# janinethoma/soft_contrastive_learning

Hardware: AMD Instinct MI355X
Metric: train-step images/sec (VGG16-NetVLAD soft-MS, 640x480) (higher is better)
Workload: dtype bf16; 1 GPU; configs[1]: wms soft-contrastive train step, VGG16-NetVLAD K=64, 24 images/GPU 640x480, bf16 backbone, float32-accurate NetVLAD + f32 loss; global_batch=24, locations=1200, parallelism=dp1, optimizer=adam

## Files before the change

### soft_contrastive_learning_amd/csrc/conv64.hip

```cpp
#include <mutex>

#include "conv_pack_layout.h"
#include "scl_common.h"

namespace {

constexpr int C64 = 64;
constexpr int TH = 8, TW = 32;
constexpr int WR = TH + 2, WC = TW + 2;
constexpr int SCR_LD = 40;
constexpr int SCR = 32 * SCR_LD;


constexpr bool kWrwBufPath = true;

constexpr int kFwSlab = 2048;
constexpr int kFwMaxSlabs = 2 * kSclMaxConvCus;
constexpr size_t kFwAux = (size_t)kFwMaxSlabs * kFwSlab, kFwAuxLen = 256;
constexpr size_t kFwStamps = kFwAux / 2, kFwCorners = kFwAux / 4 * 3;
constexpr int kFwMaxBatch = 8192;
static_assert((size_t)kSclMaxConvCus * kFwSlab <= kFwStamps, "the fused route's slabs (one per CU) end below the stamps");
static_assert(kFwStamps + (size_t)kSclMaxConvCus * 4 * 12 * 2 <= kFwCorners, "the stamps end below the corner copy");
static_assert(kFwCorners + (size_t)kFwMaxBatch * 4 * 64 / 2 <= kFwAux, "the corner copy ends below the border sums");

template <int CIN, int KOUT, int GEO = 0>
struct ConvCfg {
  static_assert(GEO == 0 || (CIN == 64 && KOUT == 64), "GEO 1 is conv1_2's geometry");
  static constexpr int TH_ = (CIN == 64 && GEO == 0) ? 8 : 4;
  static constexpr int WR_ = TH_ + 2;
  static constexpr int PIX = CIN + 8;
  static constexpr int WIN_ = WR_ * WC * PIX;
  static constexpr int PPP = CIN / 8;
  static constexpr int PIECES_ = WR_ * WC * PPP;
  static constexpr int WAVES = (CIN == 64 && KOUT == 64 && GEO == 0) ? 8 : 4;
  static constexpr int NTHR = 64 * WAVES;
  static constexpr int SPP = PPP + 1;
  static constexpr int CHUNKS = (WR_ * WC * SPP + 63) / 64;
  static constexpr int NI = (CHUNKS + WAVES - 1) / WAVES;
  static constexpr int SPT = CIN / 16;
  static constexpr int KS = 9 * SPT;
  static constexpr int NT = KOUT / 32;
  static constexpr int PARTS = WAVES / NT;
  static constexpr int MT = TH_ / PARTS;
  static constexpr size_t LDS =
      (2 * (size_t)WIN_ + WAVES * (size_t)SCR) * sizeof(unsigned short);
};

template <int CIN, int KOUT>
__global__ __launch_bounds__(256) void conv3x3_pack_kernel(const void* __restrict__ w,
                                                           int64_t sk, int64_t sc, int64_t sh,
                                                           int64_t sw, int flags,
                                                           unsigned short* __restrict__ packed) {
  using Cfg = ConvCfg<CIN, KOUT>;
  const int transposed = flags & 1, wf32 = flags & 2;
  const int idx = blockIdx.x * 256 + threadIdx.x;
  if (idx >= Cfg::NT * Cfg::KS * 512) return;
  const int64_t off = pack_src_offset(pack_reg_coord(idx, CIN), sk, sc, sh, sw, transposed);
  packed[idx] = weight_bf16(w, off, wf32);
}

template <int CIN, int KOUT, int EPI, int PL = 0, int FW = 0, int GEO = 0>
__global__ __launch_bounds__((ConvCfg<CIN, KOUT, GEO>::NTHR), (GEO ? 2 : 1)) void conv3x3_kernel(const unsigned short* __restrict__ x,
                                                         const unsigned short* __restrict__ packed,
                                                         int B, int H, int W,
                                                         unsigned short* __restrict__ out,
                                                         const float* __restrict__ bias, int relu,
                                                         unsigned short* __restrict__ pooled,
                                                         const unsigned short* __restrict__ mask,
                                                         unsigned char* __restrict__ pidx,
                                                         const unsigned char* __restrict__ uidx) {
  using Cfg = ConvCfg<CIN, KOUT, GEO>;
  constexpr int TH_ = Cfg::TH_, PIX = Cfg::PIX, WIN_ = Cfg::WIN_, KS = Cfg::KS, MT = Cfg::MT;
  static_assert(!FW || GEO == 0, "the fused first-layer gradients are written for the 8-row tile");
  extern __shared__ __attribute__((aligned(16))) unsigned short lds[];
  const int lane = threadIdx.x & 63, wid = threadIdx.x >> 6;
  const int r = lane & 31, h = lane >> 5;
  const int nt = wid % Cfg::NT, part = wid / Cfg::NT;
  unsigned short* scr = lds + 2 * WIN_ + wid * SCR;
  static_assert(!FW || (CIN == 64 && KOUT == 64 && EPI == 3 && PL == 1), "FW: conv1_2 backward-data only");
  constexpr int FWPL = 32, FGPL = TH * TW * FWPL, FXW = WR * WC * 4;
  float* dwl = reinterpret_cast<float*>(lds + 2 * WIN_ + Cfg::WAVES * SCR);
  unsigned short* xwl = reinterpret_cast<unsigned short*>(dwl + Cfg::WAVES * 1024);
  unsigned short* imc = lds + 2 * WIN_;
  const unsigned short* fx0 = reinterpret_cast<const unsigned short*>(pooled);
  float* fslabs = reinterpret_cast<float*>(pidx);
  const float bias_r = (EPI == 1 || EPI == 2 || EPI == 4) ? bias[32 * nt + r] : 0.f;
  constexpr bool SWAP = EPI == 0 || EPI == 1 || EPI == 3;
  f32x4 bias_q[4];
#pragma unroll
  for (int j = 0; j < 4; ++j)
    bias_q[j] = (SWAP && EPI == 1) ? *reinterpret_cast<const f32x4*>(bias + 32 * nt + 8 * j + 4 * h)
                                   : f32x4{0.f, 0.f, 0.f, 0.f};

  u32x4 wf[KS];
#pragma unroll
  for (int ks = 0; ks < KS; ++ks)
    wf[ks] = *reinterpret_cast<const u32x4*>(packed + (((int64_t)nt * KS + ks) * 64 + lane) * 8);

  const int tiles_x = (W + TW - 1) / TW, tiles_y = (H + TH_ - 1) / TH_;
  const int per_img = tiles_x * tiles_y;
  const int ntiles = B * per_img;

  const int wid_s = __builtin_amdgcn_readfirstlane(wid);
  int rel[Cfg::NI], roff[Cfg::NI];
#pragma unroll
  for (int i = 0; i < Cfg::NI; ++i) {
    const int slot = 64 * (wid_s + Cfg::WAVES * i) + lane;
    const int pix = slot / Cfg::SPP, piece = slot % Cfg::SPP;
    rel[i] = (piece < Cfg::PPP && pix < Cfg::WR_ * WC) ? ((pix / WC) << 8) | (pix % WC) : -1;
    roff[i] = ((pix / WC) * W + pix % WC) * CIN + 8 * piece;
  }
  const unsigned short* zeros = reinterpret_cast<const unsigned short*>(zero_block);
  auto stage_issue = [&](int tile, int buf) {
    const int b = tile / per_img, t2 = tile % per_img;
    const int y0 = (t2 / tiles_x) * TH_ - 1, x0 = (t2 % tiles_x) * TW - 1;
    const int xo = ((b * H + y0) * W + x0) * CIN;
    const unsigned base = lds_byte_of(lds) + buf * WIN_ * 2;
#pragma unroll
    for (int i = 0; i < Cfg::NI; ++i) {
      const int j = wid_s + Cfg::WAVES * i;
      if (j < Cfg::CHUNKS) {
        const int y = y0 + (rel[i] >> 8), xx = x0 + (rel[i] & 255);
        const bool ok = (unsigned)y < (unsigned)H && (unsigned)xx < (unsigned)W;
        const unsigned short* src = ok ? x + (xo + roff[i]) : zeros;
        if (rel[i] >= 0) glds16(src, base + j * 1024);
      }
    }
  };
  constexpr int PWR = TH_ / 2 + 2, PWC = TW / 2 + 2, PPP = Cfg::PPP;
  constexpr int PNR = PL ? (PWR * PWC * PPP + Cfg::NTHR - 1) / Cfg::NTHR : 1;
  constexpr int PLIVE = CIN == 64 ? 1 : PNR, NB = PNR / PLIVE, SPAN = KS / NB;
  static_assert(!PL || (PNR % PLIVE == 0 && 4 * PLIVE + 2 < SPAN), "un-pooling schedule");
  const int Ho = H >> 1, Wo = W >> 1;
  u32x4 pg[PLIVE];
  uint2 pi[PLIVE];
  const int p_piece = threadIdx.x % PPP;
  auto p_rc = [&](int rd) {
    int tid_ = threadIdx.x;
    if (FW || GEO) asm volatile("" : "+v"(tid_));
    const int pp = (tid_ + Cfg::NTHR * rd) / PPP;
    return pp < PWR * PWC ? ((pp / PWC) << 8) | (pp % PWC) : -1;
  };
  auto pool_issue = [&](int tile, int g) {
    const int b = tile / per_img, t2 = tile % per_img;
    const int py0 = (t2 / tiles_x) * (TH_ / 2) - 1, px0 = (t2 % tiles_x) * (TW / 2) - 1;
#pragma unroll
    for (int i = 0; i < PLIVE; ++i) {
      const int rc = p_rc(g * PLIVE + i);
      const int py = py0 + (rc >> 8), px = px0 + (rc & 255);
      const int off = ((b * Ho + py) * Wo + px) * CIN + 8 * p_piece;
      if (rc >= 0 && (unsigned)py < (unsigned)Ho && (unsigned)px < (unsigned)Wo) {
        pg[i] = *reinterpret_cast<const u32x4*>(x + off);
        pi[i] = *reinterpret_cast<const uint2*>(uidx + off);
      } else {
        pg[i] = u32x4{0u, 0u, 0u, 0u};
        pi[i] = uint2{0u, 0u};
      }
    }
  };
  auto pool_write = [&](int g, int i, int pos, int buf) {
    const int rc = p_rc(g * PLIVE + i);
    const int wy = 2 * (rc >> 8) + (pos >> 1) - 1, wx = 2 * (rc & 255) + (pos & 1) - 1;
    const UnpoolFlags fl = unpool_flags(pi[i].x, pi[i].y);
    const u32x4 o = unpool8(pg[i], fl, pos);
    if (rc >= 0 && (unsigned)wy < (unsigned)Cfg::WR_ && (unsigned)wx < (unsigned)WC)
      *reinterpret_cast<u32x4*>(lds + buf * WIN_ + (wy * WC + wx) * PIX + 8 * p_piece) = o;
  };

  const int dbg = SCL_DIAG_ONLY(relu >> 1);
  relu &= 1;
  const short relu_floor = relu ? (short)0 : (short)-32768;
  if ((dbg & 4) && (threadIdx.x >> 6) >= 4) __builtin_amdgcn_s_setprio(1);
  unsigned short xreg[FW ? 2 : 1];
  auto xwin_load = [&](int tile_) {
    const int b_ = tile_ / per_img, t2_ = tile_ % per_img;
    const int ty_ = (t2_ / tiles_x) * TH_, tx_ = (t2_ % tiles_x) * TW;
    int tid2 = threadIdx.x;
    asm volatile("" : "+v"(tid2));
#pragma unroll
    for (int v = 0; v < 2; ++v) {
      const int idx = v * Cfg::NTHR + tid2;
      const int pix = idx / 3, c = idx - 3 * pix;
      const int y = ty_ - 1 + pix / WC, xx = tx_ - 1 + pix % WC;
      const bool ok = idx < 3 * WR * WC && y >= 0 && y < H && xx >= 0 && xx < W;
      xreg[v] = ok ? fx0[(((int64_t)b_ * H + y) * W + xx) * 3 + c] : (unsigned short)0;
    }
  };
  auto xwin_store = [&](int par) {
    int tid2 = threadIdx.x;
    asm volatile("" : "+v"(tid2));
#pragma unroll
    for (int v = 0; v < 2; ++v) {
      const int idx = v * Cfg::NTHR + tid2;
      const int pix = idx / 3, c = idx - 3 * pix;
      if (idx < 3 * WR * WC) xwl[par * FXW + pix * 4 + c] = xreg[v];
    }
  };
  int tile = blockIdx.x;
  if (FW) {
#pragma unroll
    for (int v = 0; v < 4; ++v)
      *reinterpret_cast<f32x4*>(dwl + wid * 1024 + v * 256 + lane * 4) = f32x4{0.f, 0.f, 0.f, 0.f};
    if (tile < ntiles) {
      xwin_load(tile);
      xwin_store(0);
    }
  }
  int xpar = 0;
  uint64_t fstamp[10];
  int ftile = 0;
#define FW_STAMP(k)                                                                     \
  if (FW && (dbg & 64))                                                                 \
  asm volatile("s_memtime %0\n\ts_waitcnt lgkmcnt(0)" : "=s"(fstamp[k])::"memory")
  if (tile < ntiles) {
    if (PL) {
#pragma unroll
      for (int g = 0; g < NB; ++g) {
        pool_issue(tile, g);
#pragma unroll
        for (int sl = 0; sl < 4 * PLIVE; ++sl) pool_write(g, sl >> 2, sl & 3, 0);
      }
    } else {
      stage_issue(tile, 0);
    }
  }
  asm volatile("s_waitcnt vmcnt(0)" ::: "memory");
  __syncthreads();
  int buf = 0;
  for (; tile < ntiles; tile += gridDim.x) {
    FW_STAMP(0);
    const int next = (dbg & 1) ? ntiles : tile + gridDim.x;
    if (next < ntiles) {
      if (PL) pool_issue(next, 0); else stage_issue(next, buf ^ 1);
    }
    u32x4 mk[EPI == 3 ? MT : 1][2];
    if (EPI == 3) {
      const int b_ = tile / per_img, t2_ = tile % per_img;
      const int my0 = (t2_ / tiles_x) * TH_ + MT * part, mx = (t2_ % tiles_x) * TW + (lane >> 1);
#pragma unroll
      for (int mt = 0; mt < MT; ++mt) {
        const bool in_ = my0 + mt < H && mx < W;
        const int64_t mo = (((int64_t)b_ * H + my0 + mt) * W + mx) * KOUT + 32 * nt + 8 * (lane & 1);
        mk[mt][0] = in_ ? *reinterpret_cast<const u32x4*>(mask + mo) : u32x4{0u, 0u, 0u, 0u};
        mk[mt][1] = in_ ? *reinterpret_cast<const u32x4*>(mask + mo + 16) : u32x4{0u, 0u, 0u, 0u};
      }
    }

    const unsigned short* wb = lds + buf * WIN_ + ((MT * part) * WC + r) * PIX + 8 * h;
    f32x16 acc[MT];
#pragma unroll
    for (int mt = 0; mt < MT; ++mt) acc[mt] = zero16();
    constexpr int WRW = MT + 2, NST = Cfg::SPT * WRW * 3, RING = 4, AHEAD = 3;
    auto frag_at = [&](int st) {
      const int c = st / (WRW * 3), wr = (st / 3) % WRW, kw = st % 3;
      return *reinterpret_cast<const u32x4*>(wb + (wr * WC + kw) * PIX + 16 * c);
    };
    u32x4 af[RING];
#pragma unroll
    for (int st = 0; st < AHEAD; ++st) af[st] = frag_at(st);
#pragma unroll
    for (int st = 0; st < NST; ++st) {
      if (st + AHEAD < NST) af[(st + AHEAD) % RING] = frag_at(st + AHEAD);
      __builtin_amdgcn_sched_barrier(0);
      const int c = st / (WRW * 3), wr = (st / 3) % WRW, kw = st % 3;
#pragma unroll
      for (int mt = 0; mt < MT; ++mt) {
        const int kh = wr - mt;
        if (kh >= 0 && kh < 3)
          acc[mt] = SWAP ? mfma32b(wf[(3 * kh + kw) * Cfg::SPT + c], af[st % RING], acc[mt])
                         : mfma32b(af[st % RING], wf[(3 * kh + kw) * Cfg::SPT + c], acc[mt]);
      }
      const int ks = st * KS / NST;
      if (PL && (st == 0 || ks != (st - 1) * KS / NST)) {
        constexpr int W0 = SPAN - 4 * PLIVE - 2;
        const int g = ks / SPAN, kk = ks % SPAN;
        if (kk >= W0 && kk < W0 + 4 * PLIVE) pool_write(g, (kk - W0) >> 2, (kk - W0) & 3, buf ^ 1);
        if (kk == SPAN - 1 && g + 1 < NB && next < ntiles) pool_issue(next, g + 1);
      }
    }

    FW_STAMP(1);
    asm volatile("s_waitcnt vmcnt(0)" ::: "memory");
    FW_STAMP(2);
    if (FW) {
      __syncthreads();
      FW_STAMP(3);
      if (next < ntiles) xwin_load(next);
    }

    const int b = tile / per_img, t2 = tile % per_img;
    const int oy0 = (t2 / tiles_x) * TH_ + MT * part, ox0 = (t2 % tiles_x) * TW;
#pragma unroll
    for (int mt = 0; mt < (EPI == 4 ? 0 : MT); ++mt) {
      const int px = lane >> 1, hf = lane & 1;
      const int oy = oy0 + mt, ox = ox0 + px;
      const bool inside = oy < H && ox < W;
      const int64_t o_off = (((int64_t)b * H + oy) * W + ox) * KOUT + 32 * nt + 8 * hf;
      const u32x4 y0v = mk[EPI == 3 ? mt : 0][0], y1v = mk[EPI == 3 ? mt : 0][1];
      if (SWAP) {
#pragma unroll
        for (int j = 0; j < 4; ++j) {
          f32x4 v = {acc[mt][4 * j], acc[mt][4 * j + 1], acc[mt][4 * j + 2], acc[mt][4 * j + 3]};
          if (EPI == 1) v += bias_q[j];
          unsigned p0 = pack2_bf16(v[0], v[1]), p1 = pack2_bf16(v[2], v[3]);
          if (EPI == 1) {
            p0 = max2_i16(p0, relu_floor);
            p1 = max2_i16(p1, relu_floor);
          }
          *reinterpret_cast<uint2*>(scr + r * SCR_LD + 8 * j + 4 * h) = make_uint2(p0, p1);
        }
      } else {
#pragma unroll
        for (int q = 0; q < 16; ++q) scr[acc_row(q, h) * SCR_LD + r] = f32_to_bf16(acc[mt][q]);
      }
      __builtin_amdgcn_wave_barrier();
      u32x4 v0 = *reinterpret_cast<const u32x4*>(scr + px * SCR_LD + 8 * hf);
      u32x4 v1 = *reinterpret_cast<const u32x4*>(scr + px * SCR_LD + 8 * hf + 16);
      __builtin_amdgcn_wave_barrier();
      if (EPI == 3) {
        v0 = relu_mask(v0, y0v);
        v1 = relu_mask(v1, y1v);
      }
      if (FW && (dbg & 32)) {
      } else if (FW) {
        unsigned short* gzp = lds + buf * WIN_ + nt * FGPL + ((MT * part + mt) * TW + px) * FWPL + 8 * hf;
        *reinterpret_cast<u32x4*>(gzp) = v0;
        *reinterpret_cast<u32x4*>(gzp + 16) = v1;
        const bool cy0 = oy == 0, cy1 = oy == H - 1, cx0 = ox == 0, cx1 = ox == W - 1;
        if ((cy0 || cy1) && (cx0 || cx1)) {
          unsigned short* cp = reinterpret_cast<unsigned short*>(fslabs + kFwCorners) +
                               ((int64_t)b * 4 + (cy1 ? 2 : 0) + (cx1 ? 1 : 0)) * C64 + 32 * nt + 8 * hf;
          *reinterpret_cast<u32x4*>(cp) = v0;
          *reinterpret_cast<u32x4*>(cp + 16) = v1;
        }
      } else if (inside && !(dbg & 2)) {
        *reinterpret_cast<u32x4*>(out + o_off) = v0;
        *reinterpret_cast<u32x4*>(out + o_off + 16) = v1;
      }
    }
    if (FW) {
      FW_STAMP(4);
      __syncthreads();
      FW_STAMP(5);
      int tid2 = threadIdx.x;
      asm volatile("" : "+v"(tid2));
      const unsigned short* xw = xwl + xpar * FXW;
      const int ty_ = oy0 - MT * part, tx_ = ox0;
#pragma unroll
      for (int v = 0; v < ((dbg & 8) ? 0 : 2); ++v) {
        const int u = v * Cfg::NTHR + tid2;
        const int hh = u & 1, n = (u >> 1) & 31, s_ = u >> 6;
        const int row = s_ >> 1, col0 = 16 * (s_ & 1) + 8 * hh;
        const int nc = n < 27 ? n : 26, tap = nc / 3, c = nc - 3 * tap;
        const unsigned short* wp = xw + ((row + tap / 3) * WC + col0 + tap % 3) * 4 + c;
        unsigned e[8];
#pragma unroll
        for (int j = 0; j < 8; ++j) e[j] = wp[4 * j];
        if (n >= 27) {
          const int y = ty_ + row, xb = tx_ + col0;
          const bool rowflag = n == 27 || (n == 28 && y == 0) || (n == 29 && y == H - 1);
          const int colx = n == 30 ? 0 : (n == 31 ? W - 1 : -1);
#pragma unroll
          for (int j = 0; j < 8; ++j) e[j] = (rowflag || xb + j == colx) ? 0x3f80u : 0u;
        }
        *reinterpret_cast<u32x4*>(imc + (s_ * 32 + n) * 16 + 8 * hh) =
            u32x4{e[0] | (e[1] << 16), e[2] | (e[3] << 16), e[4] | (e[5] << 16), e[6] | (e[7] << 16)};
      }
      FW_STAMP(6);
      __syncthreads();
      FW_STAMP(7);
      int lane2 = lane, wid2 = wid;
      asm volatile("" : "+v"(lane2), "+v"(wid2));
      const int mt_ = wid2 & 1, pq = wid2 >> 1;
      const int r2 = lane2 & 31, h2 = lane2 >> 5;
      const int q4 = (lane2 >> 2) & 3, p4 = lane2 & 3, gq = lane2 >> 4;
      const unsigned short* ga = lds + buf * WIN_ + mt_ * FGPL + (8 * (gq >> 1) + q4) * FWPL +
                                 16 * (gq & 1) + 4 * p4;
      f32x16 dacc;
#pragma unroll
      for (int v = 0; v < 4; ++v) {
        const f32x4 t = *reinterpret_cast<const f32x4*>(dwl + wid2 * 1024 + v * 256 + lane2 * 4);
#pragma unroll
        for (int j = 0; j < 4; ++j) dacc[4 * v + j] = t[j];
      }
#pragma unroll
      for (int u = 0; u < ((dbg & 16) ? 0 : 4); ++u) {
        const int s_ = 4 * pq + u;
        const u32x4 a = tr_pair(ga + s_ * 16 * FWPL, 4 * FWPL);
        const u32x4 bfr = *reinterpret_cast<const u32x4*>(imc + (s_ * 32 + r2) * 16 + 8 * h2);
        dacc = mfma32b(a, bfr, dacc);
      }
#pragma unroll
      for (int v = 0; v < 4; ++v)
        *reinterpret_cast<f32x4*>(dwl + wid2 * 1024 + v * 256 + lane2 * 4) =
            f32x4{dacc[4 * v], dacc[4 * v + 1], dacc[4 * v + 2], dacc[4 * v + 3]};
      if (next < ntiles) xwin_store(xpar ^ 1);
      xpar ^= 1;
      FW_STAMP(8);
    }
    if (EPI == 2 || EPI == 4) {
      const int PH2 = H / 2, PW2 = W / 2;
      unsigned char* scr8 = reinterpret_cast<unsigned char*>(scr + 16 * SCR_LD);
#pragma unroll
      for (int mp = 0; mp < MT / 2; ++mp) {
#pragma unroll
        for (int q = 0; q < 16; q += 2) {
          const float m0 = fmaxf(acc[2 * mp][q], acc[2 * mp][q + 1]);
          const float m1 = fmaxf(acc[2 * mp + 1][q], acc[2 * mp + 1][q + 1]);
          const float m = fmaxf(m0, m1);
          scr[(acc_row(q, h) >> 1) * SCR_LD + r] = f32_to_bf16(fmaxf(m + bias_r, 0.f));
          if (EPI == 4) {
            const int k = acc[2 * mp][q] == m ? 0 : acc[2 * mp][q + 1] == m ? 1
                          : acc[2 * mp + 1][q] == m ? 2 : 3;
            scr8[(acc_row(q, h) >> 1) * 32 + r] = (unsigned char)k;
          }
        }
        __builtin_amdgcn_wave_barrier();
        const int px = lane >> 2, qu = lane & 3;
        const u32x4 v = *reinterpret_cast<const u32x4*>(scr + px * SCR_LD + 8 * qu);
        uint2 kv = uint2{0u, 0u};
        if (EPI == 4) kv = *reinterpret_cast<const uint2*>(scr8 + px * 32 + 8 * qu);
        __builtin_amdgcn_wave_barrier();
        const int py = (oy0 >> 1) + mp, pxg = (ox0 >> 1) + px;
        if (py < PH2 && pxg < PW2) {
          const int64_t po = (((int64_t)b * PH2 + py) * PW2 + pxg) * KOUT + 32 * nt + 8 * qu;
          *reinterpret_cast<u32x4*>(pooled + po) = v;
          if (EPI == 4) *reinterpret_cast<uint2*>(pidx + po) = kv;
        }
      }
    }

    __syncthreads();
    if (FW && (dbg & 64)) {
      FW_STAMP(9);
      if ((int)threadIdx.x == 64 * (dbg >> 7) && ftile >= 2 && ftile < 6) {
        uint64_t* o = reinterpret_cast<uint64_t*>(fslabs + kFwStamps) +
                      ((int64_t)blockIdx.x * 4 + (ftile - 2)) * 12;
#pragma unroll
        for (int k = 0; k < 10; ++k) o[k] = fstamp[k];
      }
      ++ftile;
    }
    buf ^= 1;
  }
#undef FW_STAMP
  if (FW) {
    __syncthreads();
    float* red = reinterpret_cast<float*>(lds);
    const int mt_ = wid & 1, pq = wid >> 1;
#pragma unroll
    for (int v = 0; v < 4; ++v) {
      const f32x4 t = *reinterpret_cast<const f32x4*>(dwl + wid * 1024 + v * 256 + lane * 4);
#pragma unroll
      for (int j = 0; j < 4; ++j) red[(pq * 64 + 32 * mt_ + acc_row(4 * v + j, h)) * 32 + r] = t[j];
    }
    __syncthreads();
    for (int e = threadIdx.x; e < kFwSlab; e += Cfg::NTHR)
      fslabs[(int64_t)blockIdx.x * kFwSlab + e] =
          (red[e] + red[kFwSlab + e]) + (red[2 * kFwSlab + e] + red[3 * kFwSlab + e]);
  }
}

constexpr int WPL = 32;
constexpr int GPLANE = TH * TW * WPL;

template <int TWv, int NKB>
struct WrwCfg {
  static constexpr int PIXELS = 256 / NKB;
  static constexpr int THv = PIXELS / TWv, WCv = TWv + 2, WRv = THv + 2;
  static constexpr int XCHv = (WRv * WCv + 15) / 16;
  static constexpr int GCHv = PIXELS / 16;
  static constexpr int XPL = XCHv * 16 * WPL, GPL = GCHv * 16 * WPL;
  static constexpr int BUF = 2 * XPL + 2 * NKB * GPL;
  static constexpr int CHUNKS = 2 * XCHv + 2 * NKB * GCHv;
  static constexpr size_t LDS = 2 * (size_t)BUF * sizeof(unsigned short);
};

template <int DBG, int TWv, int NKB, int PL = 0>
__global__ __launch_bounds__(512, 1) void wrw64_kernel(const unsigned short* __restrict__ x,
                                                       const unsigned short* __restrict__ gz,
                                                       int B, int H, int W, int C, int K,
                                                       float* __restrict__ slabs,
                                                       float* __restrict__ bslabs,
                                                       const unsigned char* __restrict__ pidx) {
  extern __shared__ __attribute__((aligned(16))) unsigned short lds[];
  const int lane = threadIdx.x & 63, wid = threadIdx.x >> 6;
  const int r = lane & 31, h = lane >> 5;
  using Cfg = WrwCfg<TWv, NKB>;
  const int n_cb = C / C64, n_kz = K / (NKB * C64), n_sib = n_cb * n_kz;
  const int n_p = gridDim.x / n_sib;
  int wg_p, wg_sib;
  if (n_p % 8 == 0) {
    const int s_ = blockIdx.x >> 3;
    wg_sib = s_ % n_sib;
    wg_p = (blockIdx.x & 7) + 8 * (s_ / n_sib);
  } else {
    wg_p = blockIdx.x % n_p;
    wg_sib = blockIdx.x / n_p;
  }
  const int wg_cb = wg_sib % n_cb, wg_kz = wg_sib / n_cb;
  constexpr int XCH = Cfg::XCHv, GCH = Cfg::GCHv, XPLANE = Cfg::XPL, GPLANE = Cfg::GPL;
  constexpr int WBUF = Cfg::BUF, WCHUNKS = Cfg::CHUNKS;
  const int mt = wid & 1, nt = NKB == 1 ? (wid >> 1) & 1 : wid >> 1, ph = NKB == 1 ? wid >> 2 : 0;
  constexpr int THv = Cfg::THv, WCv = Cfg::WCv, WRv = Cfg::WRv;
  const int q = (lane >> 2) & 3, pp = lane & 3, gq = lane >> 4;
  const int ch0 = 16 * (gq & 1) + 4 * pp;
  const int lrow = TWv == 32 ? 0 : (gq >> 1), lcol = TWv == 32 ? 8 * (gq >> 1) + q : q;

  const int tiles_x = (W + TWv - 1) / TWv, tiles_y = (H + THv - 1) / THv;
  const int per_img = tiles_x * tiles_y;
  const int ntiles = B * per_img;

  constexpr int NCH = PL ? 2 * XCH : WCHUNKS;
  constexpr int NI = (NCH + 7) / 8;
  const int wid_s = __builtin_amdgcn_readfirstlane(wid);
  const int pl = lane >> 2, piece = lane & 3;
  int rel[NI], roff[NI];
  int ldst[NI];
  bool is_x[NI];
#pragma unroll
  for (int i = 0; i < NI; ++i) {
    const int j = wid_s + 8 * i < NCH ? wid_s + 8 * i : NCH - 1;
    is_x[i] = j < 2 * XCH;
    if (j < 2 * XCH) {
      const int plane = j >= XCH ? 1 : 0;
      const int pix = 16 * (j - XCH * plane) + pl;
      rel[i] = pix < WRv * WCv ? ((pix / WCv) << 8) | (pix % WCv) : -1;
      const int pv = pix < WRv * WCv ? pix : 0;
      roff[i] = ((pv / WCv) * W + pv % WCv) * C + C64 * wg_cb + 8 * piece + 32 * plane;
      ldst[i] = (plane * XPLANE + (j - XCH * plane) * 512) * 2;
    } else {
      const int jj = j - 2 * XCH;
      const int plane = jj / GCH;
      const int pix = 16 * (jj - GCH * plane) + pl;
      rel[i] = ((pix / TWv) << 8) | (pix % TWv);
      roff[i] = ((pix / TWv) * W + pix % TWv) * K + NKB * C64 * wg_kz + 8 * piece + 32 * plane;
      ldst[i] = (2 * XPLANE + plane * GPLANE + (jj - GCH * plane) * 512) * 2;
    }
  }
  const unsigned short* zeros = reinterpret_cast<const unsigned short*>(zero_block);
  struct TilePos {
    int ty, tx, xo, go;
    int mode;
    int b, xi, gi;
  };
  auto tile_pos = [&](int tile) {
    const int b = tile / per_img, t2 = tile % per_img;
    TilePos t;
    t.ty = (t2 / tiles_x) * THv;
    t.tx = (t2 % tiles_x) * TWv;
    t.xo = ((b * H + t.ty - 1) * W + t.tx - 1) * C;
    t.go = ((b * H + t.ty) * W + t.tx) * K;
    const bool colin = t.tx >= 1 && t.tx + TWv < W;
    t.mode = __builtin_amdgcn_readfirstlane(
        colin && t.ty >= 1 && t.ty + THv < H ? 0 : (colin && kWrwBufPath && !(DBG & 8) ? 1 : 2));
    t.b = b;
    t.xi = ((t.ty - 1) * W + t.tx - 1) * C;
    t.gi = (t.ty * W + t.tx) * K;
    return t;
  };
  auto stage_chunk = [&](const TilePos& tp, int buf, int i) __attribute__((always_inline)) {
    const int ty = tp.ty, tx = tp.tx, xo = tp.xo, go = tp.go;
    const unsigned dst = __builtin_amdgcn_readfirstlane(lds_byte_of(lds) + buf * WBUF * 2 + ldst[i]);
    if (tp.mode == 0) {
      glds16_s(is_x[i] ? x + xo : gz + go, 2u * (unsigned)roff[i], dst);
    } else if (tp.mode == 1) {
      const u32x4 rs = is_x[i] ? image_rsrc(x, (int64_t)tp.b * H * W * C, (unsigned)(H * W * C) * 2u)
                               : image_rsrc(gz, (int64_t)tp.b * H * W * K, (unsigned)(H * W * K) * 2u);
      blds16(rs, 2u * (unsigned)((is_x[i] ? tp.xi : tp.gi) + roff[i]), dst);
    } else {
      const int halo = is_x[i] ? 1 : 0;
      const int y = ty - halo + (rel[i] >> 8), xx = tx - halo + (rel[i] & 255);
      const bool ok = rel[i] >= 0 && (unsigned)y < (unsigned)H && (unsigned)xx < (unsigned)W;
      const unsigned short* src = (is_x[i] ? x : gz) + ((is_x[i] ? xo : go) + roff[i]);
      glds16(ok ? src : zeros, dst);
    }
  };
  auto stage_issue = [&](int tile, int buf) __attribute__((always_inline)) {
    const TilePos tp = tile_pos(tile);
#pragma unroll
    for (int i = 0; i < NI; ++i) stage_chunk(tp, buf, i);
  };
  constexpr int NPC = TWv / 2, NPR = THv / 2;
  const int p_piece = threadIdx.x & 3, p_pc = (threadIdx.x >> 2) % NPC;
  const int p_pr = ((threadIdx.x >> 2) / NPC) % NPR, p_plane = (threadIdx.x >> 2) / (NPC * NPR);
  const int Ho = H >> 1, Wo = W >> 1;
  u32x4 pg = {0u, 0u, 0u, 0u};
  uint2 pi = {0u, 0u};
  auto pool_issue = [&](int tile) {
    const int b = tile / per_img, t2 = tile % per_img;
    const int py = (t2 / tiles_x) * NPR + p_pr, px = (t2 % tiles_x) * NPC + p_pc;
    const int off = ((b * Ho + py) * Wo + px) * K + NKB * C64 * wg_kz + 32 * p_plane + 8 * p_piece;
    if (py < Ho && px < Wo) {
      pg = *reinterpret_cast<const u32x4*>(gz + off);
      pi = *reinterpret_cast<const uint2*>(pidx + off);
    } else {
      pg = u32x4{0u, 0u, 0u, 0u};
      pi = uint2{0u, 0u};
    }
  };
  auto pool_write = [&](int buf) {
    unsigned short* dst = lds + buf * WBUF + 2 * XPLANE + p_plane * GPLANE +
                          (2 * p_pr * TWv + 2 * p_pc) * WPL + 8 * p_piece;
    const UnpoolFlags fl = unpool_flags(pi.x, pi.y);
#pragma unroll
    for (int pos = 0; pos < 4; ++pos)
      *reinterpret_cast<u32x4*>(dst + ((pos >> 1) * TWv + (pos & 1)) * WPL) = unpool8(pg, fl, pos);
  };

  f32x16 acc[9];
#pragma unroll
  for (int t = 0; t < 9; ++t) acc[t] = zero16();
  float bsum = 0.f;
  typedef __bf16 bf16x2 __attribute__((ext_vector_type(2)));

  uint64_t stamp[7];
#define WRW_STAMP(k)                                                   \
  if (DBG & 4) asm volatile("s_memtime %0\n\ts_waitcnt lgkmcnt(0)" : "=s"(stamp[k])::"memory")
  int tile = wg_p;
  if (tile < ntiles) {
    stage_issue(tile, 0);
    if (PL) {
      pool_issue(tile);
      pool_write(0);
    }
  }
  asm volatile("s_waitcnt vmcnt(0)" ::: "memory");
  __syncthreads();
  int buf = 0, tcount = 0;
  for (; tile < ntiles; tile += n_p) {
    WRW_STAMP(0);
    const int next = (DBG & 2) ? ntiles : tile + n_p;
    const TilePos stg = tile_pos(next < ntiles ? next : tile);
    if (PL && next < ntiles) pool_issue(next);
    WRW_STAMP(1);
    const unsigned short* xl =
        lds + buf * WBUF + mt * XPLANE + (lrow * WCv + lcol) * WPL + ch0;
    const unsigned short* gl =
        lds + buf * WBUF + 2 * XPLANE + nt * GPLANE + (lrow * TWv + lcol) * WPL + ch0;
    struct XFrag {
      uint2 lo, hi, ex;
    };
    auto x_frag = [&](int wrow, int cx) {
      const unsigned short* p = xl + (wrow * WCv + cx) * WPL;
      XFrag f;
      f.lo = __builtin_bit_cast(uint2, lds_tr16(p));
      f.hi = __builtin_bit_cast(uint2, lds_tr16(p + 4 * WPL));
      f.ex = __builtin_bit_cast(uint2, lds_tr16(p + 8 * WPL));
      return f;
    };
    constexpr int NFR = TWv == 32 ? 6 : 18, NFC = TWv == 32 ? 2 : 1;
    auto f_row = [](int s_, int kh) { return TWv == 32 ? (s_ & 3) + kh : 2 * s_ + kh; };
    auto f_col = [](int s_) { return TWv == 32 ? (s_ >> 2) : 0; };
    auto f_first = [](int s_, int kh) { return TWv == 32 ? ((s_ & 3) == 0 || kh == 2) : (s_ == 0 || kh >= 1); };
    const int row_w = TWv == 32 ? 4 * ph : 16 * ph;
    XFrag fr[NFR][NFC];
    auto f_load = [&](int i) {
      const int s_ = i / 9, kh = (i % 9) / 3;
      fr[f_row(s_, kh)][f_col(s_)] = x_frag(row_w + f_row(s_, kh), 16 * f_col(s_));
    };
    auto b_of = [&](int s_) {
      const int ry = TWv == 32 ? 4 * ph + (s_ & 3) : 16 * ph + 2 * s_;
      return tr_pair(gl + (ry * TWv + 16 * f_col(s_)) * WPL, 4 * WPL);
    };
    constexpr int LEAD = 6;
    constexpr int STG = 5;
    static_assert(STG * NI <= 9 * 8 - 12, "the last chunk needs time to land");
    u32x4 bf[2];
#pragma unroll
    for (int i = 0; i < LEAD; i += 3)
      if (f_first(i / 9, (i % 9) / 3)) f_load(i);
    bf[0] = b_of(0);
#pragma unroll
    for (int i = 0; i < 9 * 8; ++i) {
      const int s_ = i / 9, kh = (i % 9) / 3, kw = i % 3;
      if (i + LEAD < 9 * 8 && (i + LEAD) % 3 == 0 && f_first((i + LEAD) / 9, ((i + LEAD) % 9) / 3))
        f_load(i + LEAD);
      if (i % 9 == 2 && s_ + 1 < 8) bf[(s_ + 1) & 1] = b_of(s_ + 1);
      if (!(DBG & 2) && i % STG == 0 && i / STG < NI) stage_chunk(stg, buf ^ 1, i / STG);
      __builtin_amdgcn_sched_barrier(0);
      const XFrag& f = fr[f_row(s_, kh)][f_col(s_)];
      u32x4 a;
      if (kw == 0)
        a = u32x4{f.lo.x, f.lo.y, f.hi.x, f.hi.y};
      else if (kw == 1)
        a = u32x4{__builtin_amdgcn_alignbit(f.lo.y, f.lo.x, 16), __builtin_amdgcn_alignbit(f.hi.x, f.lo.y, 16),
                  __builtin_amdgcn_alignbit(f.hi.y, f.hi.x, 16), __builtin_amdgcn_alignbit(f.ex.x, f.hi.y, 16)};
      else
        a = u32x4{f.lo.y, f.hi.x, f.hi.y, f.ex.x};
      if constexpr ((DBG & 16) != 0) {
        f32x16& c_ = acc[i % 9];
        const int o_ = 8 * (i & 1);
        f32x4 q0 = {c_[o_], c_[o_ + 1], c_[o_ + 2], c_[o_ + 3]};
        f32x4 q1 = {c_[o_ + 4], c_[o_ + 5], c_[o_ + 6], c_[o_ + 7]};
        q0 = mfma16b(a, bf[s_ & 1], q0);
        q1 = mfma16b(a, bf[s_ & 1], q1);
        c_[o_] = q0[0]; c_[o_ + 1] = q0[1]; c_[o_ + 2] = q0[2]; c_[o_ + 3] = q0[3];
        c_[o_ + 4] = q1[0]; c_[o_ + 5] = q1[1]; c_[o_ + 6] = q1[2]; c_[o_ + 7] = q1[3];
      } else {
        acc[i % 9] = mfma32b(a, bf[s_ & 1], acc[i % 9]);
      }
      if (i == 8) WRW_STAMP(2);
      if (i == 35) WRW_STAMP(3);
      if (i == 71) WRW_STAMP(4);
      if (i % 9 == 4) {
        const u32x4 bw = bf[s_ & 1];
        const bf16x2 one2 = __builtin_bit_cast(bf16x2, 0x3f803f80u);
        const unsigned w0 = bw.x, w1 = bw.y, w2 = bw.z, w3 = bw.w;
        bsum = __builtin_amdgcn_fdot2_f32_bf16(__builtin_bit_cast(bf16x2, w0), one2, bsum, false);
        bsum = __builtin_amdgcn_fdot2_f32_bf16(__builtin_bit_cast(bf16x2, w1), one2, bsum, false);
        bsum = __builtin_amdgcn_fdot2_f32_bf16(__builtin_bit_cast(bf16x2, w2), one2, bsum, false);
        bsum = __builtin_amdgcn_fdot2_f32_bf16(__builtin_bit_cast(bf16x2, w3), one2, bsum, false);
      }
    }
    if (PL && next < ntiles) pool_write(buf ^ 1);
    asm volatile("s_waitcnt vmcnt(0)" ::: "memory");
    WRW_STAMP(5);
    __syncthreads();
    WRW_STAMP(6);
    if (DBG & 4) {
      asm volatile("s_waitcnt lgkmcnt(0)" ::: "memory");
      if (threadIdx.x == 0 && tcount < 4) {
        uint64_t* o = reinterpret_cast<uint64_t*>(bslabs) + ((int64_t)((int)blockIdx.x) * 4 + tcount) * 8;
#pragma unroll
        for (int k = 0; k < 7; ++k) o[k] = stamp[k];
      }
      ++tcount;
    }
    buf ^= 1;
  }
#undef WRW_STAMP

  const int slab = NKB == 1 ? 2 * wg_p + ph : wg_p;
  const int kb = NKB == 1 ? wg_kz : 2 * wg_kz + (nt >> 1);
  float* out = slabs + (((int64_t)slab * n_cb + wg_cb) * (NKB * n_kz) + kb) * 9 * C64 * C64;
#pragma unroll
  for (int t = 0; t < 9; ++t)
#pragma unroll
    for (int qq = 0; qq < 16; ++qq)
      out[(t * C64 + 32 * mt + acc_row(qq, h)) * C64 + 32 * (nt & 1) + r] = acc[t][qq];
  const float bs = bsum + __shfl_xor(bsum, 32);
  if (bslabs && !(DBG & 4) && wg_cb == 0 && mt == 0 && h == 0)
// ... 1075 lines not shown
```

Measured before the change: 2039 images/sec.

## Feed fused conv1_1 weight-gradient MFMA from registers instead of LDS staging

In the fused conv1_2 backward-data plus conv1_1 weight-gradient path, the ReLU-masked gradient is now packed straight from the accumulators into MFMA A-operands held in registers, using per-wave mask bits computed early with packed integer min/max ops. This removes the LDS round trip, the transpose reads and two block barriers per tile. The im2col tile build is split into chunks claimed dynamically through an LDS atomic counter, and the input-window indexing is precomputed once per thread. It also issues the next tile's input load earlier and skips the trailing vmcnt wait, at the cost of more register pressure and more intricate corner-copy logic.

```diff
diff --git a/soft_contrastive_learning_amd/csrc/conv64.hip b/soft_contrastive_learning_amd/csrc/conv64.hip
--- a/soft_contrastive_learning_amd/csrc/conv64.hip
+++ b/soft_contrastive_learning_amd/csrc/conv64.hip
@@ -22,6 +22,22 @@
 static_assert((size_t)kSclMaxConvCus * kFwSlab <= kFwStamps, "the fused route's slabs (one per CU) end below the stamps");
 static_assert(kFwStamps + (size_t)kSclMaxConvCus * 4 * 12 * 2 <= kFwCorners, "the stamps end below the corner copy");
 static_assert(kFwCorners + (size_t)kFwMaxBatch * 4 * 64 / 2 <= kFwAux, "the corner copy ends below the border sums");
+
+__device__ __forceinline__ unsigned positive_bits(u32x4 y) {
+  unsigned k[4];
+#pragma unroll
+  for (int i = 0; i < 4; ++i) {
+    asm("v_pk_max_i16 %0, %1, 0" : "=v"(k[i]) : "v"(y[i]));
+    asm("v_pk_min_i16 %0, %1, 1 op_sel_hi:[1,0]" : "=v"(k[i]) : "v"(k[i]));
+  }
+  const unsigned t = k[0] | (k[1] << 2) | (k[2] << 4) | (k[3] << 6);
+  return t | (t >> 15);
+}
+__device__ __forceinline__ unsigned keep_halves(unsigned g, unsigned keep) {
+  unsigned out;
+  asm("v_pk_mul_lo_u16 %0, %1, %2" : "=v"(out) : "v"(g), "v"(keep));
+  return out;
+}
 
 template <int CIN, int KOUT, int GEO = 0>
 struct ConvCfg {
@@ -78,14 +94,17 @@
   const int nt = wid % Cfg::NT, part = wid / Cfg::NT;
   unsigned short* scr = lds + 2 * WIN_ + wid * SCR;
   static_assert(!FW || (CIN == 64 && KOUT == 64 && EPI == 3 && PL == 1), "FW: conv1_2 backward-data only");
-  constexpr int FWPL = 32, FGPL = TH * TW * FWPL, FXW = WR * WC * 4;
+  constexpr int FXW = WR * WC * 4;
   float* dwl = reinterpret_cast<float*>(lds + 2 * WIN_ + Cfg::WAVES * SCR);
   unsigned short* xwl = reinterpret_cast<unsigned short*>(dwl + Cfg::WAVES * 1024);
+  constexpr int IMC = 16 * 32 * 16;
+  static_assert(!FW || (size_t)IMC * 2 + Cfg::WAVES * 256 + 4 <= (size_t)Cfg::WAVES * SCR * 2, "im2col tile + mask bits + counter fit the scratch");
   unsigned short* imc = lds + 2 * WIN_;
+  unsigned* icnt = reinterpret_cast<unsigned*>(imc + IMC + Cfg::WAVES * 128);
   const unsigned short* fx0 = reinterpret_cast<const unsigned short*>(pooled);
   float* fslabs = reinterpret_cast<float*>(pidx);
   const float bias_r = (EPI == 1 || EPI == 2 || EPI == 4) ? bias[32 * nt + r] : 0.f;
-  constexpr bool SWAP = EPI == 0 || EPI == 1 || EPI == 3;
+  constexpr bool SWAP = (EPI == 0 || EPI == 1 || EPI == 3) && !FW;
   f32x4 bias_q[4];
 #pragma unroll
   for (int j = 0; j < 4; ++j)
@@ -172,42 +191,45 @@
   const short relu_floor = relu ? (short)0 : (short)-32768;
   if ((dbg & 4) && (threadIdx.x >> 6) >= 4) __builtin_amdgcn_s_setprio(1);
   unsigned short xreg[FW ? 2 : 1];
+  int xrel[FW ? 2 : 1], xpk[FW ? 2 : 1];
+  if (FW) {
+#pragma unroll
+    for (int v = 0; v < 2; ++v) {
+      const int idx = v * Cfg::NTHR + (int)threadIdx.x;
+      const int pix = idx / 3, c = idx - 3 * pix;
+      xrel[v] = ((pix / WC) * W + pix % WC) * 3 + c;
+      xpk[v] = idx < 3 * WR * WC ? ((pix * 4 + c) << 16) | ((pix / WC) << 8) | (pix % WC) : -1;
+    }
+  }
   auto xwin_load = [&](int tile_) {
     const int b_ = tile_ / per_img, t2_ = tile_ % per_img;
     const int ty_ = (t2_ / tiles_x) * TH_, tx_ = (t2_ % tiles_x) * TW;
-    int tid2 = threadIdx.x;
-    asm volatile("" : "+v"(tid2));
+    const int base = ((b_ * H + ty_ - 1) * W + tx_ - 1) * 3;
 #pragma unroll
     for (int v = 0; v < 2; ++v) {
-      const int idx = v * Cfg::NTHR + tid2;
-      const int pix = idx / 3, c = idx - 3 * pix;
-      const int y = ty_ - 1 + pix / WC, xx = tx_ - 1 + pix % WC;
-      const bool ok = idx < 3 * WR * WC && y >= 0 && y < H && xx >= 0 && xx < W;
-      xreg[v] = ok ? fx0[(((int64_t)b_ * H + y) * W + xx) * 3 + c] : (unsigned short)0;
+      const int y = ty_ - 1 + ((xpk[v] >> 8) & 255), xx = tx_ - 1 + (xpk[v] & 255);
+      const bool ok = xpk[v] >= 0 && (unsigned)y < (unsigned)H && (unsigned)xx < (unsigned)W;
+      xreg[v] = ok ? fx0[base + xrel[v]] : (unsigned short)0;
     }
   };
   auto xwin_store = [&](int par) {
-    int tid2 = threadIdx.x;
-    asm volatile("" : "+v"(tid2));
-#pragma unroll
-    for (int v = 0; v < 2; ++v) {
-      const int idx = v * Cfg::NTHR + tid2;
-      const int pix = idx / 3, c = idx - 3 * pix;
-      if (idx < 3 * WR * WC) xwl[par * FXW + pix * 4 + c] = xreg[v];
-    }
+#pragma unroll
+    for (int v = 0; v < 2; ++v)
+      if (xpk[v] >= 0) xwl[par * FXW + (xpk[v] >> 16)] = xreg[v];
   };
   int tile = blockIdx.x;
   if (FW) {
 #pragma unroll
     for (int v = 0; v < 4; ++v)
       *reinterpret_cast<f32x4*>(dwl + wid * 1024 + v * 256 + lane * 4) = f32x4{0.f, 0.f, 0.f, 0.f};
+    if (threadIdx.x == 0) *icnt = 0u;
     if (tile < ntiles) {
       xwin_load(tile);
       xwin_store(0);
     }
   }
-  int xpar = 0;
-  uint64_t fstamp[10];
+  int xpar = 0, fti = 0;
+  uint64_t fstamp[8];
   int ftile = 0;
 #define FW_STAMP(k)                                                                     \
   if (FW && (dbg & 64))                                                                 \
@@ -277,21 +299,31 @@
         if (kk >= W0 && kk < W0 + 4 * PLIVE) pool_write(g, (kk - W0) >> 2, (kk - W0) & 3, buf ^ 1);
         if (kk == SPAN - 1 && g + 1 < NB && next < ntiles) pool_issue(next, g + 1);
       }
+      if (FW && ks != (st - 1) * KS / NST) {
+        if (ks == KS - 2 && !(dbg & 32)) {
+          int lane2 = lane, wid2 = wid;
+          asm volatile("" : "+v"(lane2), "+v"(wid2));
+          const int mpx = lane2 >> 1, mhf = lane2 & 1;
+          unsigned char* mw = reinterpret_cast<unsigned char*>(imc + IMC) + wid2 * 256 +
+                              (2 * mhf + ((mpx >> 2) & 1)) * 16 + 4 * (mpx >> 3) + 2 * (mpx & 1) + ((mpx >> 1) & 1);
+#pragma unroll
+          for (int mt = 0; mt < MT; ++mt) {
+            mw[mt * 128] = (unsigned char)positive_bits(mk[mt][0]);
+            mw[mt * 128 + 64] = (unsigned char)positive_bits(mk[mt][1]);
+          }
+        }
+        if (ks == KS - 1 && next < ntiles) xwin_load(next);
+      }
     }
 
     FW_STAMP(1);
-    asm volatile("s_waitcnt vmcnt(0)" ::: "memory");
+    if (!FW) asm volatile("s_waitcnt vmcnt(0)" ::: "memory");
     FW_STAMP(2);
-    if (FW) {
-      __syncthreads();
-      FW_STAMP(3);
-      if (next < ntiles) xwin_load(next);
-    }
 
     const int b = tile / per_img, t2 = tile % per_img;
     const int oy0 = (t2 / tiles_x) * TH_ + MT * part, ox0 = (t2 % tiles_x) * TW;
 #pragma unroll
-    for (int mt = 0; mt < (EPI == 4 ? 0 : MT); ++mt) {
+    for (int mt = 0; mt < ((EPI == 4 || FW) ? 0 : MT); ++mt) {
       const int px = lane >> 1, hf = lane & 1;
       const int oy = oy0 + mt, ox = ox0 + px;
       const bool inside = oy < H && ox < W;
@@ -321,61 +353,86 @@
         v0 = relu_mask(v0, y0v);
         v1 = relu_mask(v1, y1v);
       }
-      if (FW && (dbg & 32)) {
-      } else if (FW) {
-        unsigned short* gzp = lds + buf * WIN_ + nt * FGPL + ((MT * part + mt) * TW + px) * FWPL + 8 * hf;
-        *reinterpret_cast<u32x4*>(gzp) = v0;
-        *reinterpret_cast<u32x4*>(gzp + 16) = v1;
-        const bool cy0 = oy == 0, cy1 = oy == H - 1, cx0 = ox == 0, cx1 = ox == W - 1;
-        if ((cy0 || cy1) && (cx0 || cx1)) {
-          unsigned short* cp = reinterpret_cast<unsigned short*>(fslabs + kFwCorners) +
-                               ((int64_t)b * 4 + (cy1 ? 2 : 0) + (cx1 ? 1 : 0)) * C64 + 32 * nt + 8 * hf;
-          *reinterpret_cast<u32x4*>(cp) = v0;
-          *reinterpret_cast<u32x4*>(cp + 16) = v1;
-        }
-      } else if (inside && !(dbg & 2)) {
+      if (inside && !(dbg & 2)) {
         *reinterpret_cast<u32x4*>(out + o_off) = v0;
         *reinterpret_cast<u32x4*>(out + o_off + 16) = v1;
       }
     }
     if (FW) {
-      FW_STAMP(4);
-      __syncthreads();
-      FW_STAMP(5);
-      int tid2 = threadIdx.x;
-      asm volatile("" : "+v"(tid2));
+      int lane2 = lane, wid2 = wid;
+      asm volatile("" : "+v"(lane2), "+v"(wid2));
+      const int mt_ = wid2 & 1, pq = wid2 >> 1;
+      const int r2 = lane2 & 31, h2 = lane2 >> 5;
+      const int ty_ = (t2 / tiles_x) * TH_, tx_ = ox0;
+      u32x4 ga[MT][2];
+      {
+        const unsigned char* mb = reinterpret_cast<const unsigned char*>(imc + IMC) + wid2 * 256;
+        __builtin_amdgcn_wave_barrier();
+#pragma unroll
+        for (int mt = 0; mt < MT; ++mt) {
+          u32x4 mbits = u32x4{~0u, ~0u, ~0u, ~0u};
+          if (!(dbg & 32)) mbits = *reinterpret_cast<const u32x4*>(mb + mt * 128 + (2 * (r2 >> 3) + h2) * 16);
+          unsigned w[8];
+#pragma unroll
+          for (int d = 0; d < 4; ++d) {
+            const unsigned m = mbits[d] >> (r2 & 7);
+            w[2 * d] = keep_halves(pack2_bf16(acc[mt][4 * d], acc[mt][4 * d + 1]), m & 0x00010001u);
+            w[2 * d + 1] = keep_halves(pack2_bf16(acc[mt][4 * d + 2], acc[mt][4 * d + 3]), (m >> 8) & 0x00010001u);
+          }
+          ga[mt][0] = u32x4{w[0], w[1], w[2], w[3]};
+          ga[mt][1] = u32x4{w[4], w[5], w[6], w[7]};
+        }
+        __builtin_amdgcn_wave_barrier();
+        const int cy_ = ty_ + MT * (__builtin_amdgcn_readfirstlane(wid2) >> 1);
+#pragma unroll
+        for (int mt = 0; mt < MT; ++mt) {
+          const int oy = cy_ + mt;
+          if (oy == 0 || oy == H - 1) {
+            unsigned short* cp = reinterpret_cast<unsigned short*>(fslabs + kFwCorners) +
+                                 ((int64_t)b * 4 + (oy == H - 1 ? 2 : 0)) * C64 + 32 * mt_ + r2;
+            if (ox0 == 0 && h2 == 0) cp[0] = (unsigned short)(ga[mt][0].x & 0xffffu);
+            const int cpx = W - 1 - ox0;
+            if (cpx >= 0 && cpx < TW) {
+              const int cq = 4 * (cpx >> 3) + (cpx & 3);
+              unsigned cw = 0;
+#pragma unroll
+              for (int k = 0; k < 8; ++k) {
+                const unsigned wk = k < 4 ? ga[mt][0][k] : ga[mt][1][k - 4];
+                cw = (cq >> 1) == k ? wk : cw;
+              }
+              if (((cpx >> 2) & 1) == h2) cp[C64] = (unsigned short)((cq & 1) ? cw >> 16 : cw & 0xffffu);
+            }
+          }
+        }
+      }
+      FW_STAMP(3);
       const unsigned short* xw = xwl + xpar * FXW;
-      const int ty_ = oy0 - MT * part, tx_ = ox0;
-#pragma unroll
-      for (int v = 0; v < ((dbg & 8) ? 0 : 2); ++v) {
-        const int u = v * Cfg::NTHR + tid2;
-        const int hh = u & 1, n = (u >> 1) & 31, s_ = u >> 6;
-        const int row = s_ >> 1, col0 = 16 * (s_ & 1) + 8 * hh;
+      while (!(dbg & 8)) {
+        unsigned claim = 0;
+        if (lane2 == 0) claim = atomicAdd(icnt, 1u);
+        const int s_ = __builtin_amdgcn_readfirstlane(claim) - 24 * fti;
+        if ((unsigned)s_ >= 16u) break;
+        const int hh = lane2 & 1, n = lane2 >> 1;
+        const int row = s_ >> 1, col0 = 16 * (s_ & 1) + 4 * hh;
         const int nc = n < 27 ? n : 26, tap = nc / 3, c = nc - 3 * tap;
         const unsigned short* wp = xw + ((row + tap / 3) * WC + col0 + tap % 3) * 4 + c;
         unsigned e[8];
 #pragma unroll
-        for (int j = 0; j < 8; ++j) e[j] = wp[4 * j];
+        for (int j = 0; j < 8; ++j) e[j] = wp[4 * (8 * (j >> 2) + (j & 3))];
         if (n >= 27) {
           const int y = ty_ + row, xb = tx_ + col0;
           const bool rowflag = n == 27 || (n == 28 && y == 0) || (n == 29 && y == H - 1);
           const int colx = n == 30 ? 0 : (n == 31 ? W - 1 : -1);
 #pragma unroll
-          for (int j = 0; j < 8; ++j) e[j] = (rowflag || xb + j == colx) ? 0x3f80u : 0u;
+          for (int j = 0; j < 8; ++j) e[j] = (rowflag || xb + 8 * (j >> 2) + (j & 3) == colx) ? 0x3f80u : 0u;
         }
         *reinterpret_cast<u32x4*>(imc + (s_ * 32 + n) * 16 + 8 * hh) =
             u32x4{e[0] | (e[1] << 16), e[2] | (e[3] << 16), e[4] | (e[5] << 16), e[6] | (e[7] << 16)};
       }
-      FW_STAMP(6);
+      ++fti;
+      FW_STAMP(4);
       __syncthreads();
-      FW_STAMP(7);
-      int lane2 = lane, wid2 = wid;
-      asm volatile("" : "+v"(lane2), "+v"(wid2));
-      const int mt_ = wid2 & 1, pq = wid2 >> 1;
-      const int r2 = lane2 & 31, h2 = lane2 >> 5;
-      const int q4 = (lane2 >> 2) & 3, p4 = lane2 & 3, gq = lane2 >> 4;
-      const unsigned short* ga = lds + buf * WIN_ + mt_ * FGPL + (8 * (gq >> 1) + q4) * FWPL +
-                                 16 * (gq & 1) + 4 * p4;
+      FW_STAMP(5);
       f32x16 dacc;
 #pragma unroll
       for (int v = 0; v < 4; ++v) {
@@ -386,9 +443,8 @@
 #pragma unroll
       for (int u = 0; u < ((dbg & 16) ? 0 : 4); ++u) {
         const int s_ = 4 * pq + u;
-        const u32x4 a = tr_pair(ga + s_ * 16 * FWPL, 4 * FWPL);
         const u32x4 bfr = *reinterpret_cast<const u32x4*>(imc + (s_ * 32 + r2) * 16 + 8 * h2);
-        dacc = mfma32b(a, bfr, dacc);
+        dacc = mfma32b(ga[u >> 1][u & 1], bfr, dacc);
       }
 #pragma unroll
       for (int v = 0; v < 4; ++v)
@@ -396,7 +452,7 @@
             f32x4{dacc[4 * v], dacc[4 * v + 1], dacc[4 * v + 2], dacc[4 * v + 3]};
       if (next < ntiles) xwin_store(xpar ^ 1);
       xpar ^= 1;
-      FW_STAMP(8);
+      FW_STAMP(6);
     }
     if (EPI == 2 || EPI == 4) {
       const int PH2 = H / 2, PW2 = W / 2;
@@ -432,12 +488,12 @@
 
     __syncthreads();
     if (FW && (dbg & 64)) {
-      FW_STAMP(9);
+      FW_STAMP(7);
       if ((int)threadIdx.x == 64 * (dbg >> 7) && ftile >= 2 && ftile < 6) {
         uint64_t* o = reinterpret_cast<uint64_t*>(fslabs + kFwStamps) +
                       ((int64_t)blockIdx.x * 4 + (ftile - 2)) * 12;
 #pragma unroll
-        for (int k = 0; k < 10; ++k) o[k] = fstamp[k];
+        for (int k = 0; k < 8; ++k) o[k] = fstamp[k];
       }
       ++ftile;
     }
```

Measured after the change: 2048 images/sec, median of 5. No clear change (+0.4%).
